# aws-neuron/neuronx-distributed

Measured on AMD Instinct MI355X. Metric: tokens/sec (whole node) Llama-2-7B training, TP=num_gpus, seq=4096, higher is better.
Workload: dtype bf16; 1 GPU; model=llama2-7b, global_batch=32, seq_len=4096, parallelism=tp1, zero1=True

## Files before the change

neuronx_distributed_amd/ops/__init__.py:

```python

import ctypes
import math
import os
from typing import Optional

import torch

_LIB = None
_LIB_ERR = None


def _load():
    global _LIB, _LIB_ERR
    if _LIB is not None or _LIB_ERR is not None:
        return _LIB
    from .build import LIB

    if not os.path.exists(LIB):
        _LIB_ERR = f"{LIB} not built — run neuronx_distributed_amd.ops.build"
        return None
    try:
        lib = ctypes.CDLL(LIB)
    except OSError as e:
        _LIB_ERR = str(e)
# ... 312 lines not shown
            dx = torch.empty_like(x)
            lib.swiglu_bwd(_ptr(x), _ptr(dy2), _ptr(dx), ctypes.c_long(N),
                           ctypes.c_int(I), _stream())
            return dx
        g, u = x[..., :I].float(), x[..., I:].float()
        dyf = dy.float()
        sig = torch.sigmoid(g)
        s = g * sig
        dg = dyf * u * (sig + s * (1 - sig))
        du = dyf * s
        return torch.cat([dg, du], dim=-1).to(x.dtype)


def swiglu(x: torch.Tensor) -> torch.Tensor:
    return _SwiGLUFn.apply(x)



def flash_attn_available() -> bool:
    lib = _load()
    return lib is not None and hasattr(lib, "flash_attn_fwd")


def _fa_ok_layout(t) -> bool:
    return t.stride(3) == 1


def _fa_strides(*tensors):
    vals = []
    for t in tensors:
        vals += [t.stride(0), t.stride(1), t.stride(2)]
    arr = (ctypes.c_long * len(vals))(*vals)
    return arr


def _fa_alloc_like(t):
    B, H, S, D = t.shape
    if t.stride(1) == D and t.stride(2) == H * D:
        return torch.empty(B, S, H, D, dtype=t.dtype,
                           device=t.device).permute(0, 2, 1, 3)
    return torch.empty_like(t, memory_format=torch.contiguous_format)


class _FlashAttnFn(torch.autograd.Function):
    @staticmethod
    def forward(ctx, q, k, v, causal, scale, window=0):
        lib = _require_lib()
        B, Hq, S, D = q.shape
        Hkv = k.shape[1]
        assert D == 128, "flash kernel supports D=128"
        assert q.dtype == torch.bfloat16
        if not _fa_ok_layout(q):
            q = q.contiguous()
        if not _fa_ok_layout(k):
            k = k.contiguous()
        if not _fa_ok_layout(v):
            v = v.contiguous()
        out = _fa_alloc_like(q)
        lse = torch.empty(B, Hq, S, dtype=torch.float32, device=q.device)
        lib.flash_attn_fwd_strided(
            _ptr(q), _ptr(k), _ptr(v), _ptr(out), _ptr(lse),
            ctypes.c_int(B), ctypes.c_int(Hq), ctypes.c_int(Hkv),
            ctypes.c_int(S), ctypes.c_float(scale),
            ctypes.c_int(1 if causal else 0), ctypes.c_int(window or 0),
            _fa_strides(q, k, v, out), _stream())
        ctx.save_for_backward(q, k, v, out, lse)
        ctx.causal = causal
        ctx.scale = scale
        ctx.window = window or 0
        return out

    @staticmethod
    def backward(ctx, dout):
        q, k, v, out, lse = ctx.saved_tensors
        lib = _require_lib()
        if not hasattr(lib, "flash_attn_bwd"):
            raise RuntimeError("flash_attn_bwd kernel not built")
        B, Hq, S, D = q.shape
        Hkv = k.shape[1]
        if not _fa_ok_layout(dout):
            dout = dout.contiguous()
        delta = torch.empty(B, Hq, S, dtype=torch.float32, device=q.device)
        dq = _fa_alloc_like(q)
        dk_pq = torch.empty(B, Hq, S, D, dtype=q.dtype, device=q.device)
        dv_pq = torch.empty(B, Hq, S, D, dtype=q.dtype, device=q.device)
        lib.flash_attn_bwd_strided(
            _ptr(q), _ptr(k), _ptr(v), _ptr(out), _ptr(dout),
            _ptr(lse), _ptr(delta), _ptr(dq), _ptr(dk_pq), _ptr(dv_pq),
            ctypes.c_int(B), ctypes.c_int(Hq), ctypes.c_int(Hkv),
            ctypes.c_int(S), ctypes.c_float(ctx.scale),
            ctypes.c_int(1 if ctx.causal else 0),
            ctypes.c_int(getattr(ctx, "window", 0)),
            _fa_strides(q, k, v, out, dout, dq, dk_pq, dv_pq), _stream())
        rep = Hq // Hkv
        if rep > 1:
            dk = dk_pq.view(B, Hkv, rep, S, D).float().sum(2).to(q.dtype)
            dv = dv_pq.view(B, Hkv, rep, S, D).float().sum(2).to(q.dtype)
        else:
            dk = dk_pq
            dv = dv_pq
        return dq, dk, dv, None, None, None


def flash_attn(q, k, v, causal=True, softmax_scale=None, window=0):
    scale = softmax_scale or 1.0 / math.sqrt(q.shape[-1])
    return _FlashAttnFn.apply(q, k, v, causal, scale, window)


def flash_attn_window_available() -> bool:
    lib = _load()
    return lib is not None and hasattr(lib, "flash_attn_fwd_window")


def flash_attn_windowed(q, k, v, window: int, softmax_scale=None):
    lib = _require_lib()
    B, Hq, S, D = q.shape
    Hkv = k.shape[1]
    assert D == 128 and q.dtype == torch.bfloat16
    scale = softmax_scale or 1.0 / math.sqrt(D)
    q, k, v = q.contiguous(), k.contiguous(), v.contiguous()
    out = torch.empty_like(q)
    lse = torch.empty(B, Hq, S, dtype=torch.float32, device=q.device)
    lib.flash_attn_fwd_window(_ptr(q), _ptr(k), _ptr(v), _ptr(out),
                              _ptr(lse), ctypes.c_int(B), ctypes.c_int(Hq),
                              ctypes.c_int(Hkv), ctypes.c_int(S),
                              ctypes.c_float(scale), ctypes.c_int(window),
                              _stream())
    return out



def adamw_step(master: torch.Tensor, m: torch.Tensor, v: torch.Tensor,
               grad_bf16: torch.Tensor, param_bf16: torch.Tensor,
               clip: Optional[torch.Tensor], lr: float, beta1: float,
               beta2: float, eps: float, weight_decay: float, step: int):
    lib = _require_lib()
    n = master.numel()
    assert m.numel() == n and v.numel() == n and grad_bf16.numel() == n
    assert grad_bf16.dtype == torch.bfloat16 and param_bf16.dtype == torch.bfloat16
    inv_bc1 = 1.0 / (1.0 - beta1 ** step)
    inv_bc2 = 1.0 / (1.0 - beta2 ** step)
    lib.adamw_step(ctypes.c_long(n), _ptr(master), _ptr(m), _ptr(v),
                   _ptr(grad_bf16), _ptr(param_bf16),
                   _ptr(clip) if clip is not None else None,
                   ctypes.c_float(lr), ctypes.c_float(beta1),
                   ctypes.c_float(beta2), ctypes.c_float(eps),
                   ctypes.c_float(weight_decay), ctypes.c_float(inv_bc1),
                   ctypes.c_float(inv_bc2), _stream())



_MOE_MB = 16


def moe_decode_available() -> bool:
    lib = _load()
    return lib is not None and hasattr(lib, "moe_decode_glu")


def moe_decode_glu(hidden: torch.Tensor, gate_up_w: torch.Tensor,
                   down_w: torch.Tensor, expert_affinities: torch.Tensor,
                   expert_index: torch.Tensor) -> torch.Tensor:
    lib = _require_lib()
    T, H = hidden.shape
    E, _, twoI = gate_up_w.shape
    I = twoI // 2
    assert H % 64 == 0 and I % 64 == 0, (H, I)
    k = expert_index.shape[1]
# ... 104 lines not shown
```

neuronx_distributed_amd/ops/csrc/flash_attn_bwd.hip:

```cpp

#include "common.h"
#include "mfma.h"

#define TR_PITCH 40

#define FA_D 128
#define LOG2E 1.4426950408889634f

extern "C" __global__ void __launch_bounds__(256)
fa_bwd_delta_kernel(const short* __restrict__ dout,
                    const short* __restrict__ out, float* __restrict__ delta,
                    long rows, int Hq, int S,
                    long do_bs, long do_hs, long do_ss,
                    long o_bs, long o_hs, long o_ss) {
  const int sub = threadIdx.x & 15;
  const long row0 = ((long)blockIdx.x * blockDim.x + threadIdx.x) >> 4;
  const long row_step = ((long)gridDim.x * blockDim.x) >> 4;
  for (long row = row0; row < rows; row += row_step) {
    const long b = row / ((long)Hq * S);
    const long h = (row / S) % Hq;
    const long sq = row % S;
    s8v dv = *(const s8v*)(dout + b * do_bs + h * do_hs + sq * do_ss
                           + sub * 8);
    s8v ov = *(const s8v*)(out + b * o_bs + h * o_hs + sq * o_ss + sub * 8);
    float s = 0.f;
#pragma unroll
    for (int j = 0; j < 8; ++j) s += bits2f(dv[j]) * bits2f(ov[j]);
#pragma unroll
    for (int off = 8; off >= 1; off >>= 1) s += __shfl_xor(s, off, 64);
    if (sub == 0) delta[row] = s;
  }
}



struct StageRegs { uint4v v0, v1; };

__device__ __forceinline__ StageRegs load_tile32(const short* __restrict__ src,
                                                 long src_row0,
                                                 long src_stride,
                                                 int rows_valid) {
  int rp = (threadIdx.x & 255) >> 4;
  int c16 = threadIdx.x & 15;
  int r0 = 2 * rp, r1 = 2 * rp + 1;
  int rr0 = r0 < rows_valid ? r0 : (rows_valid > 0 ? rows_valid - 1 : 0);
  int rr1 = r1 < rows_valid ? r1 : (rows_valid > 0 ? rows_valid - 1 : 0);
  StageRegs r;
  r.v0 = *(const uint4v*)(src + (src_row0 + rr0) * src_stride + c16 * 8);
  r.v1 = *(const uint4v*)(src + (src_row0 + rr1) * src_stride + c16 * 8);
  return r;
}

__device__ __forceinline__ void write_tile32(StageRegs r, char* lds_rm,
                                             char* lds_tr) {
  if (blockDim.x > 256 && threadIdx.x >= 256) return;
  int rp = threadIdx.x >> 4;
  int c16 = threadIdx.x & 15;
  int r0 = 2 * rp, r1 = 2 * rp + 1;
  *(uint4v*)(lds_rm + r0 * (FA_D * 2) + swz16(r0, c16 * 16)) = r.v0;
  *(uint4v*)(lds_rm + r1 * (FA_D * 2) + swz16(r1, c16 * 16)) = r.v1;
  union { uint4v u; short s[8]; } a, b;
  a.u = r.v0; b.u = r.v1;
#pragma unroll
  for (int j = 0; j < 8; ++j) {
    int d = c16 * 8 + j;
    uint pair = ((uint)(unsigned short)a.s[j]) |
                (((uint)(unsigned short)b.s[j]) << 16);
    *(uint*)(lds_tr + d * (TR_PITCH * 2) + r0 * 2) = pair;
  }
}

__device__ __forceinline__ void write_tile32_rm(StageRegs r, char* lds_rm) {
  if (blockDim.x > 256 && threadIdx.x >= 256) return;
  int rp = threadIdx.x >> 4;
  int c16 = threadIdx.x & 15;
  int r0 = 2 * rp, r1 = 2 * rp + 1;
  *(uint4v*)(lds_rm + r0 * (FA_D * 2) + swz16(r0, c16 * 16)) = r.v0;
  *(uint4v*)(lds_rm + r1 * (FA_D * 2) + swz16(r1, c16 * 16)) = r.v1;
}

__device__ __forceinline__ void stage_tile32(const short* __restrict__ src,
                                             long src_row0, long src_stride,
                                             int rows_valid, char* lds_rm,
                                             char* lds_tr) {
  if (blockDim.x > 256 && threadIdx.x >= 256) return;
  int rp = threadIdx.x >> 4;
  int c16 = threadIdx.x & 15;
  int r0 = 2 * rp, r1 = 2 * rp + 1;
  int rr0 = r0 < rows_valid ? r0 : (rows_valid > 0 ? rows_valid - 1 : 0);
  int rr1 = r1 < rows_valid ? r1 : (rows_valid > 0 ? rows_valid - 1 : 0);
  uint4v v0 = *(const uint4v*)(src + (src_row0 + rr0) * src_stride + c16 * 8);
  uint4v v1 = *(const uint4v*)(src + (src_row0 + rr1) * src_stride + c16 * 8);
  *(uint4v*)(lds_rm + r0 * (FA_D * 2) + swz16(r0, c16 * 16)) = v0;
  *(uint4v*)(lds_rm + r1 * (FA_D * 2) + swz16(r1, c16 * 16)) = v1;
  union { uint4v u; short s[8]; } a, b;
  a.u = v0; b.u = v1;
#pragma unroll
  for (int j = 0; j < 8; ++j) {
    int d = c16 * 8 + j;
    uint pair = ((uint)(unsigned short)a.s[j]) |
                (((uint)(unsigned short)b.s[j]) << 16);
    *(uint*)(lds_tr + d * (TR_PITCH * 2) + r0 * 2) = pair;
  }
}

#define TR_TILE_B (FA_D * TR_PITCH * 2)

#define TR64_PITCH 72
#define TR64_TILE_B (FA_D * TR64_PITCH * 2)
#define BW64_LDS_Q 0
#define BW64_LDS_DO (64 * FA_D * 2)
#define BW64_LDS_QT (2 * 64 * FA_D * 2)
#define BW64_LDS_DOT (2 * 64 * FA_D * 2 + TR64_TILE_B)
#define BW64_LDS_LD (2 * 64 * FA_D * 2 + 2 * TR64_TILE_B)
#define BW64_LDS_X (BW64_LDS_LD + 128 * 4)
#define BW64_X_SLOT(kvg, half, f) \
  ((((kvg) * 2 + (half)) * 4 + (f)) * 64 * 16)

struct Stage64Regs { uint4v v0, v1; };

__device__ __forceinline__ Stage64Regs load_tile64(
    const short* __restrict__ src, long src_row0, long src_stride,
    int rows_valid) {
  int rp = threadIdx.x >> 4;
  int c16 = threadIdx.x & 15;
  int r0 = 2 * rp, r1 = 2 * rp + 1;
  int rr0 = r0 < rows_valid ? r0 : (rows_valid > 0 ? rows_valid - 1 : 0);
  int rr1 = r1 < rows_valid ? r1 : (rows_valid > 0 ? rows_valid - 1 : 0);
  Stage64Regs r;
  r.v0 = *(const uint4v*)(src + (src_row0 + rr0) * src_stride + c16 * 8);
  r.v1 = *(const uint4v*)(src + (src_row0 + rr1) * src_stride + c16 * 8);
  return r;
}

__device__ __forceinline__ void write_tile64(Stage64Regs r, char* lds_rm,
                                             char* lds_tr) {
  int rp = threadIdx.x >> 4;
  int c16 = threadIdx.x & 15;
  int r0 = 2 * rp, r1 = 2 * rp + 1;
  *(uint4v*)(lds_rm + r0 * (FA_D * 2) + swz16(r0, c16 * 16)) = r.v0;
  *(uint4v*)(lds_rm + r1 * (FA_D * 2) + swz16(r1, c16 * 16)) = r.v1;
  union { uint4v u; short s[8]; } a, b;
  a.u = r.v0; b.u = r.v1;
#pragma unroll
  for (int j = 0; j < 8; ++j) {
    int d = c16 * 8 + j;
    uint pair = ((uint)(unsigned short)a.s[j]) |
                (((uint)(unsigned short)b.s[j]) << 16);
    *(uint*)(lds_tr + d * (TR64_PITCH * 2) + r0 * 2) = pair;
  }
}

__device__ __forceinline__ void stage_tile64(const short* __restrict__ src,
                                             long src_row0, long src_stride,
                                             int rows_valid, char* lds_rm,
                                             char* lds_tr) {
  write_tile64(load_tile64(src, src_row0, src_stride, rows_valid), lds_rm,
               lds_tr);
}

extern "C" __global__ void __launch_bounds__(512, 2)
fa_bwd_dkdv_kernel(const short* __restrict__ qp, const short* __restrict__ kp,
                   const short* __restrict__ vp,
                   const short* __restrict__ dop,
                   const float* __restrict__ lsep,
                   const float* __restrict__ deltap,
                   short* __restrict__ dkp, short* __restrict__ dvp,
                   int B, int Hq, int Hkv, int S, float scale, int causal,
                   int window,
                   long q_bs, long q_hs, long q_ss,
                   long k_bs, long k_hs, long k_ss,
                   long v_bs, long v_hs, long v_ss,
                   long do_bs, long do_hs, long do_ss,
                   long dk_bs, long dk_hs, long dk_ss,
                   long dv_bs, long dv_hs, long dv_ss) {
  extern __shared__ __attribute__((aligned(16))) char smem[];
  const int lane = threadIdx.x & 63;
  const int wid = __builtin_amdgcn_readfirstlane(threadIdx.x >> 6);
  const int col = lane & 31;
  const int hi = lane >> 5;
  const int kvg = wid >> 1;
  const int dhalf = wid & 1;

  const int kvblk = blockIdx.y;
  const int h = blockIdx.x;
  const int b = blockIdx.z;
  const int hkv = h / (Hq / Hkv);
  const long q_base = (long)b * q_bs + (long)h * q_hs;
  const long do_base = (long)b * do_bs + (long)h * do_hs;
  const long k_base = (long)b * k_bs + (long)hkv * k_hs;
  const long v_base = (long)b * v_bs + (long)hkv * v_hs;
  const long lse_base = (long)(b * Hq + h) * S;

  const int kv0 = kvblk * 128 + kvg * 32;
  const int my_k = kv0 + col;

  frag_u kf[8], vf[8];
  {
    int row = my_k < S ? my_k : S - 1;
#pragma unroll
    for (int c = 0; c < 8; ++c) {
      kf[c].u4 = *(const uint4v*)(kp + k_base + (long)row * k_ss + c * 16 + hi * 8);
      vf[c].u4 = *(const uint4v*)(vp + v_base + (long)row * v_ss + c * 16 + hi * 8);
    }
  }

  f32x16 dv_acc[2] = {};
  f32x16 dk_acc[2] = {};

  float* ld_sm = (float*)(smem + BW64_LDS_LD);
  auto load_ld = [&](int qt0) -> float {
    int qg = qt0 + (threadIdx.x & 63);
    int qc = qg < S ? qg : S - 1;
    if (threadIdx.x < 64) return lsep[lse_base + qc] * LOG2E;
    if (threadIdx.x < 128) return deltap[lse_base + qc];
    return 0.f;
  };
  auto write_ld = [&](float v) {
    if (threadIdx.x < 128) ld_sm[threadIdx.x] = v;
  };

  const float s2 = scale * LOG2E;
  int q_start = causal ? kvblk * 128 : 0;
  int q_end = S;
  if (window > 0) {
    int qe = kvblk * 128 + 127 + window;
    q_end = qe < S ? qe : S;
  }

  stage_tile64(qp + q_base, q_start, q_ss, S - q_start, smem + BW64_LDS_Q,
               smem + BW64_LDS_QT);
  stage_tile64(dop + do_base, q_start, do_ss, S - q_start, smem + BW64_LDS_DO,
               smem + BW64_LDS_DOT);
  write_ld(load_ld(q_start));

  Stage64Regs nq, ndo;
  float nld = 0.f;
  for (int q0 = q_start; q0 < q_end; q0 += 64) {
    __syncthreads();
    if (q0 + 64 < q_end) {
      nq = load_tile64(qp + q_base, q0 + 64, q_ss, S - q0 - 64);
      ndo = load_tile64(dop + do_base, q0 + 64, do_ss, S - q0 - 64);
      nld = load_ld(q0 + 64);
    }
    {
      const int half = dhalf;
      const int qh0 = q0 + half * 32;
      const bool produce =
          (!causal || (qh0 + 31 >= kv0)) && qh0 < S &&
          (window <= 0 || qh0 < kv0 + 31 + window);
      if (produce) {
        const int rm_row = half * 32 + col;
        const int my_kv = kv0 + col;

        f32x16 st = {};
        f32x16 dpt = {};
#pragma unroll
        for (int c = 0; c < 8; ++c) {
          frag_u qfr, dofr;
          qfr.u4 = *(const uint4v*)(smem + BW64_LDS_Q + rm_row * (FA_D * 2)
                                    + swz16(rm_row, (c * 16 + hi * 8) * 2));
          st = mfma_bf16(qfr.bf, kf[c].bf, st);
          dofr.u4 = *(const uint4v*)(smem + BW64_LDS_DO + rm_row * (FA_D * 2)
                                     + swz16(rm_row, (c * 16 + hi * 8) * 2));
          dpt = mfma_bf16(dofr.bf, vf[c].bf, dpt);
        }

        float lse_v[16], dlt_v[16];
#pragma unroll
        for (int g = 0; g < 4; ++g) {
          *(float4*)(lse_v + 4 * g) =
              *(const float4*)(ld_sm + half * 32 + 8 * g + 4 * hi);
          *(float4*)(dlt_v + 4 * g) =
              *(const float4*)(ld_sm + 64 + half * 32 + 8 * g + 4 * hi);
        }
#pragma unroll
        for (int r = 0; r < 16; ++r) {
          int ql = half * 32 + acc_row(r, hi);
          int qg = q0 + ql;
          bool masked = (causal && my_kv > qg) || my_kv >= S || qg >= S ||
              (window > 0 && qg >= my_kv + window);
          float p =
              masked ? 0.f : __builtin_amdgcn_exp2f(st[r] * s2 - lse_v[r]);
          st[r] = p;
          dpt[r] = p * (dpt[r] - dlt_v[r]);
        }

        frag_u pA[2], dA[2];
#pragma unroll
        for (int cc = 0; cc < 2; ++cc) {
          uint b0 = pack_bf16x2(st[8 * cc + 0], st[8 * cc + 1]);
          uint b1 = pack_bf16x2(st[8 * cc + 2], st[8 * cc + 3]);
          uint b2 = pack_bf16x2(st[8 * cc + 4], st[8 * cc + 5]);
          uint b3 = pack_bf16x2(st[8 * cc + 6], st[8 * cc + 7]);
          {
            auto r01 = __builtin_amdgcn_permlane32_swap(b0, b2, false, false);
            b0 = r01[0]; b2 = r01[1];
          }
          {
            auto r23 = __builtin_amdgcn_permlane32_swap(b1, b3, false, false);
            b1 = r23[0]; b3 = r23[1];
          }
          pA[cc].u[0] = b0; pA[cc].u[1] = b1;
          pA[cc].u[2] = b2; pA[cc].u[3] = b3;
          uint c0 = pack_bf16x2(dpt[8 * cc + 0], dpt[8 * cc + 1]);
          uint c1 = pack_bf16x2(dpt[8 * cc + 2], dpt[8 * cc + 3]);
          uint c2 = pack_bf16x2(dpt[8 * cc + 4], dpt[8 * cc + 5]);
          uint c3 = pack_bf16x2(dpt[8 * cc + 6], dpt[8 * cc + 7]);
          {
            auto r01 = __builtin_amdgcn_permlane32_swap(c0, c2, false, false);
            c0 = r01[0]; c2 = r01[1];
          }
          {
            auto r23 = __builtin_amdgcn_permlane32_swap(c1, c3, false, false);
            c1 = r23[0]; c3 = r23[1];
          }
          dA[cc].u[0] = c0; dA[cc].u[1] = c1;
          dA[cc].u[2] = c2; dA[cc].u[3] = c3;
        }

        char* xb = smem + BW64_LDS_X;
        *(uint4v*)(xb + BW64_X_SLOT(kvg, half, 0) + lane * 16) = pA[0].u4;
        *(uint4v*)(xb + BW64_X_SLOT(kvg, half, 1) + lane * 16) = pA[1].u4;
        *(uint4v*)(xb + BW64_X_SLOT(kvg, half, 2) + lane * 16) = dA[0].u4;
        *(uint4v*)(xb + BW64_X_SLOT(kvg, half, 3) + lane * 16) = dA[1].u4;
      }
    }
    __syncthreads();

#pragma unroll
    for (int half = 0; half < 2; ++half) {
      const int qh0 = q0 + half * 32;
      if ((causal && qh0 + 31 < kv0) || qh0 >= S ||
          (window > 0 && qh0 >= kv0 + 31 + window)) continue;

      frag_u dofr[2][2], qfr2[2][2];
#pragma unroll
      for (int cq = 0; cq < 2; ++cq)
#pragma unroll
        for (int nb = 0; nb < 2; ++nb) {
          int d = dhalf * 64 + nb * 32 + col;
          dofr[cq][nb].u4 = *(const uint4v*)(smem + BW64_LDS_DOT
                                             + d * (TR64_PITCH * 2)
                                             + (half * 32 + cq * 16 + hi * 8) * 2);
          qfr2[cq][nb].u4 = *(const uint4v*)(smem + BW64_LDS_QT
                                             + d * (TR64_PITCH * 2)
                                             + (half * 32 + cq * 16 + hi * 8) * 2);
        }
      frag_u pA[2], dA[2];
      const char* xb = smem + BW64_LDS_X;
      pA[0].u4 = *(const uint4v*)(xb + BW64_X_SLOT(kvg, half, 0) + lane * 16);
      pA[1].u4 = *(const uint4v*)(xb + BW64_X_SLOT(kvg, half, 1) + lane * 16);
      dA[0].u4 = *(const uint4v*)(xb + BW64_X_SLOT(kvg, half, 2) + lane * 16);
      dA[1].u4 = *(const uint4v*)(xb + BW64_X_SLOT(kvg, half, 3) + lane * 16);

      __builtin_amdgcn_s_setprio(1);
#pragma unroll
      for (int cq = 0; cq < 2; ++cq)
#pragma unroll
        for (int nb = 0; nb < 2; ++nb) {
          dv_acc[nb] = mfma_bf16(pA[cq].bf, dofr[cq][nb].bf, dv_acc[nb]);
          dk_acc[nb] = mfma_bf16(dA[cq].bf, qfr2[cq][nb].bf, dk_acc[nb]);
        }
      __builtin_amdgcn_s_setprio(0);
    }

    __syncthreads();
    if (q0 + 64 < q_end) {
      write_tile64(nq, smem + BW64_LDS_Q, smem + BW64_LDS_QT);
      write_tile64(ndo, smem + BW64_LDS_DO, smem + BW64_LDS_DOT);
      write_ld(nld);
    }
  }

  __syncthreads();
  char* otile = smem + wid * (32 * 64 * 2);
#pragma unroll
  for (int nb = 0; nb < 2; ++nb)
#pragma unroll
    for (int r = 0; r < 16; ++r) {
      int k = acc_row(r, hi);
      int dd = nb * 32 + col;
      *(short*)(otile + (k * 64 + dd) * 2) = f2bits(dv_acc[nb][r]);
    }
  __builtin_amdgcn_s_waitcnt(0);
#pragma unroll
  for (int i = 0; i < 4; ++i) {
    int p = lane + i * 64;
    int row = p >> 3, c16 = p & 7;
    int kg = kv0 + row;
    if (kg < S) {
      uint4v vv = *(const uint4v*)(otile + (row * 64 + c16 * 8) * 2);
      *(uint4v*)(dvp + (long)b * dv_bs + (long)h * dv_hs
                 + (long)kg * dv_ss + dhalf * 64
                 + c16 * 8) = vv;
    }
  }
  __builtin_amdgcn_s_waitcnt(0);
#pragma unroll
  for (int nb = 0; nb < 2; ++nb)
#pragma unroll
    for (int r = 0; r < 16; ++r) {
      int k = acc_row(r, hi);
      int dd = nb * 32 + col;
      *(short*)(otile + (k * 64 + dd) * 2) = f2bits(dk_acc[nb][r] * scale);
    }
  __builtin_amdgcn_s_waitcnt(0);
#pragma unroll
  for (int i = 0; i < 4; ++i) {
    int p = lane + i * 64;
    int row = p >> 3, c16 = p & 7;
    int kg = kv0 + row;
    if (kg < S) {
      uint4v vv = *(const uint4v*)(otile + (row * 64 + c16 * 8) * 2);
      *(uint4v*)(dkp + (long)b * dk_bs + (long)h * dk_hs
                 + (long)kg * dk_ss + dhalf * 64
                 + c16 * 8) = vv;
    }
  }
}

#define DQ_LDS_K 0
#define DQ_LDS_KT (32 * FA_D * 2)
#define DQ_LDS_V (32 * FA_D * 2 + TR_TILE_B)

extern "C" __global__ void __launch_bounds__(256, 2)
fa_bwd_dq_kernel(const short* __restrict__ qp, const short* __restrict__ kp,
                 const short* __restrict__ vp, const short* __restrict__ dop,
                 const float* __restrict__ lsep,
                 const float* __restrict__ deltap, short* __restrict__ dqp,
                 int B, int Hq, int Hkv, int S, float scale, int causal,
                 int window,
                 long q_bs, long q_hs, long q_ss,
                 long k_bs, long k_hs, long k_ss,
                 long v_bs, long v_hs, long v_ss,
                 long do_bs, long do_hs, long do_ss,
                 long dq_bs, long dq_hs, long dq_ss) {
  extern __shared__ __attribute__((aligned(16))) char smem[];
  const int lane = threadIdx.x & 63;
  const int wid = __builtin_amdgcn_readfirstlane(threadIdx.x >> 6);
  const int col = lane & 31;
  const int hi = lane >> 5;

  const int qblk = (int)(gridDim.y - 1 - blockIdx.y);
  const int h = blockIdx.x;
  const int b = blockIdx.z;
  const int hkv = h / (Hq / Hkv);
  const long q_base = (long)b * q_bs + (long)h * q_hs;
  const long do_base = (long)b * do_bs + (long)h * do_hs;
  const long dq_base = (long)b * dq_bs + (long)h * dq_hs;
  const long k_base = (long)b * k_bs + (long)hkv * k_hs;
  const long v_base = (long)b * v_bs + (long)hkv * v_hs;
  const long lse_base = (long)(b * Hq + h) * S;

  const int q0 = qblk * 128 + wid * 32;
  const int my_q = q0 + col;
  const int q_ld = my_q < S ? my_q : S - 1;

  frag_u qf[8], dof[8];
#pragma unroll
  for (int c = 0; c < 8; ++c) {
    qf[c].u4 = *(const uint4v*)(qp + q_base + (long)q_ld * q_ss + c * 16 + hi * 8);
    dof[c].u4 = *(const uint4v*)(dop + do_base + (long)q_ld * do_ss + c * 16 + hi * 8);
  }
  const float lse2 = lsep[lse_base + q_ld] * LOG2E;
  const float dlt = deltap[lse_base + q_ld];

  f32x16 dq_acc[4] = {};

  const int kv_end = causal ? min(S, qblk * 128 + 128) : S;
  const int kv_begin = window > 0
      ? ((qblk * 128 - window + 1 > 0 ? qblk * 128 - window + 1 : 0) & ~31)
      : 0;
  const float s2 = scale * LOG2E;

  stage_tile32(kp + k_base, kv_begin, k_ss, S - kv_begin, smem + DQ_LDS_K,
               smem + DQ_LDS_KT);
  write_tile32_rm(load_tile32(vp + v_base, kv_begin, v_ss, S - kv_begin),
                  smem + DQ_LDS_V);

  StageRegs nk, nv;
  for (int kv0 = kv_begin; kv0 < kv_end; kv0 += 32) {
    __syncthreads();
    if (kv0 + 32 < kv_end) {
      nk = load_tile32(kp + k_base, kv0 + 32, k_ss, S - kv0 - 32);
      nv = load_tile32(vp + v_base, kv0 + 32, v_ss, S - kv0 - 32);
    }
    const bool wave_active = (!causal || (kv0 <= q0 + 31)) &&
        (window <= 0 || kv0 + 31 + window > q0);

    if (wave_active) {
      f32x16 st = {};
      f32x16 dpt = {};
#pragma unroll
      for (int c = 0; c < 8; ++c) {
        frag_u kfr;
        kfr.u4 = *(const uint4v*)(smem + DQ_LDS_K + col * (FA_D * 2)
                                  + swz16(col, (c * 16 + hi * 8) * 2));
        st = mfma_bf16(kfr.bf, qf[c].bf, st);
        frag_u vfr;
        vfr.u4 = *(const uint4v*)(smem + DQ_LDS_V + col * (FA_D * 2)
                                  + swz16(col, (c * 16 + hi * 8) * 2));
        dpt = mfma_bf16(vfr.bf, dof[c].bf, dpt);
      }

      f32x16 dst;
#pragma unroll
      for (int r = 0; r < 16; ++r) {
        int kg = kv0 + acc_row(r, hi);
        bool masked = (causal && kg > my_q) || kg >= S || my_q >= S ||
            (window > 0 && kg <= my_q - window);
        float p = masked ? 0.f : __builtin_amdgcn_exp2f(st[r] * s2 - lse2);
        dst[r] = p * (dpt[r] - dlt);
      }

      frag_u kfr2[2][4];
#pragma unroll
      for (int ck = 0; ck < 2; ++ck)
#pragma unroll
        for (int nb = 0; nb < 4; ++nb) {
          int d = nb * 32 + col;
          kfr2[ck][nb].u4 = *(const uint4v*)(smem + DQ_LDS_KT
                                             + d * (TR_PITCH * 2)
                                             + (ck * 16 + hi * 8) * 2);
        }

      frag_u dA[2];
#pragma unroll
      for (int cc = 0; cc < 2; ++cc) {
        uint b0 = pack_bf16x2(dst[8 * cc + 0], dst[8 * cc + 1]);
        uint b1 = pack_bf16x2(dst[8 * cc + 2], dst[8 * cc + 3]);
        uint b2 = pack_bf16x2(dst[8 * cc + 4], dst[8 * cc + 5]);
        uint b3 = pack_bf16x2(dst[8 * cc + 6], dst[8 * cc + 7]);
        {
          auto r01 = __builtin_amdgcn_permlane32_swap(b0, b2, false, false);
          b0 = r01[0]; b2 = r01[1];
        }
        {
          auto r23 = __builtin_amdgcn_permlane32_swap(b1, b3, false, false);
          b1 = r23[0]; b3 = r23[1];
        }
        dA[cc].u[0] = b0; dA[cc].u[1] = b1;
        dA[cc].u[2] = b2; dA[cc].u[3] = b3;
      }

      __builtin_amdgcn_s_setprio(1);
#pragma unroll
      for (int ck = 0; ck < 2; ++ck) {
#pragma unroll
        for (int nb = 0; nb < 4; ++nb) {
          dq_acc[nb] = mfma_bf16(dA[ck].bf, kfr2[ck][nb].bf, dq_acc[nb]);
        }
      }
      __builtin_amdgcn_s_setprio(0);
    }

    __syncthreads();
    if (kv0 + 32 < kv_end) {
      write_tile32(nk, smem + DQ_LDS_K, smem + DQ_LDS_KT);
      write_tile32_rm(nv, smem + DQ_LDS_V);
    }
  }

  __syncthreads();
  char* otile = smem + wid * (32 * FA_D * 2);
#pragma unroll
  for (int nb = 0; nb < 4; ++nb)
#pragma unroll
    for (int r = 0; r < 16; ++r) {
      int qr = acc_row(r, hi);
      int d = nb * 32 + col;
      *(short*)(otile + (qr * FA_D + d) * 2) = f2bits(dq_acc[nb][r] * scale);
    }
  __builtin_amdgcn_s_waitcnt(0);
#pragma unroll
  for (int i = 0; i < 8; ++i) {
    int p = lane + i * 64;
    int row = p >> 4, c16 = p & 15;
    int qg = q0 + row;
    if (qg < S) {
      uint4v vv = *(const uint4v*)(otile + (row * FA_D + c16 * 8) * 2);
      *(uint4v*)(dqp + dq_base + (long)qg * dq_ss + c16 * 8) = vv;
    }
  }
}

extern "C" void flash_attn_bwd_strided(
    const void* q, const void* k, const void* v, const void* out,
    const void* dout, const void* lse, void* delta, void* dq, void* dk,
    void* dv, int B, int Hq, int Hkv, int S, float scale, int causal,
    int window, const long* st, hipStream_t stream) {
  long rows = (long)B * Hq * S;
  long blocks = (rows + 15) / 16;
  int nb = blocks < 8192 ? (int)blocks : 8192;
  fa_bwd_delta_kernel<<<nb, 256, 0, stream>>>(
      (const short*)dout, (const short*)out, (float*)delta, rows, Hq, S,
      st[12], st[13], st[14], st[9], st[10], st[11]);
  dim3 gkv(Hq, (S + 127) / 128, B);
  size_t lds1 = BW64_LDS_X + 8 * 4 * 64 * 16;
  fa_bwd_dkdv_kernel<<<gkv, 512, lds1, stream>>>(
      (const short*)q, (const short*)k, (const short*)v, (const short*)dout,
      (const float*)lse, (const float*)delta, (short*)dk, (short*)dv, B, Hq,
      Hkv, S, scale, causal, window, st[0], st[1], st[2], st[3], st[4],
      st[5], st[6], st[7], st[8], st[12], st[13], st[14], st[18], st[19],
      st[20], st[21], st[22], st[23]);
  dim3 gq(Hq, (S + 127) / 128, B);
  size_t lds2 = 4 * 32 * FA_D * 2;
  fa_bwd_dq_kernel<<<gq, 256, lds2, stream>>>(
      (const short*)q, (const short*)k, (const short*)v, (const short*)dout,
      (const float*)lse, (const float*)delta, (short*)dq, B, Hq, Hkv, S,
      scale, causal, window, st[0], st[1], st[2], st[3], st[4], st[5],
      st[6], st[7], st[8], st[12], st[13], st[14], st[15], st[16],
      st[17]);
}

extern "C" void flash_attn_bwd(const void* q, const void* k, const void* v,
                               const void* out, const void* dout,
                               const void* lse, void* delta, void* dq,
                               void* dk, void* dv, int B, int Hq, int Hkv,
                               int S, float scale, int causal,
                               hipStream_t stream) {
  const long qd[3] = {(long)Hq * S * FA_D, (long)S * FA_D, FA_D};
  const long kd[3] = {(long)Hkv * S * FA_D, (long)S * FA_D, FA_D};
  long st[24];
  for (int i = 0; i < 3; ++i) {
    st[0 + i] = qd[i];
    st[3 + i] = kd[i];
    st[6 + i] = kd[i];
    st[9 + i] = qd[i];
    st[12 + i] = qd[i];
    st[15 + i] = qd[i];
    st[18 + i] = qd[i];
    st[21 + i] = qd[i];
  }
  flash_attn_bwd_strided(q, k, v, out, dout, lse, delta, dq, dk, dv, B, Hq,
                         Hkv, S, scale, causal, 0, st, stream);
}
```

neuronx_distributed_amd/ops/csrc/mfma.h:

```cpp
#pragma once

#include "common.h"

typedef __bf16 bf16x8 __attribute__((ext_vector_type(8)));
typedef float f32x16 __attribute__((ext_vector_type(16)));
typedef unsigned int uint4v __attribute__((ext_vector_type(4)));

__device__ __forceinline__ f32x16 mfma_bf16(bf16x8 a, bf16x8 b, f32x16 c) {
  return __builtin_amdgcn_mfma_f32_32x32x16_bf16(a, b, c, 0, 0, 0);
}

union frag_u {
  bf16x8 bf;
  uint4v u4;
  uint u[4];
};

__device__ __forceinline__ int acc_row(int r, int hi) {
  return (r & 3) + 8 * (r >> 2) + 4 * hi;
}

__device__ __forceinline__ uint pack_bf16x2(float lo, float hi) {
  union { __bf16 b[2]; uint u; } r;
  r.b[0] = (__bf16)lo;
  r.b[1] = (__bf16)hi;
  return r.u;
}

__device__ __forceinline__ int swz(int row, int byte_in_row) {
  return byte_in_row ^ ((row & 7) << 4);
}

__device__ __forceinline__ int swz16(int row, int byte_in_row) {
  return byte_in_row ^ ((row & 15) << 4);
}
```

Before: 21730 tokens/s.

## Use single swizzled LDS image with transpose reads and double-buffer attention backward tiles

Replaces the separate row-major and explicitly transposed LDS copies in the flash-attention backward kernels with one swizzled tile image. Transposed operands are read with ds_read_tr16_b64, and staging buffers are double-buffered so one __syncthreads per iteration can be dropped. The dq kernel moves from 32-row to 64-row KV tiles, and masking is skipped for tiles that need no mask. It also avoids allocating per-query-head dk/dv buffers when Hq == Hkv. The aim is to cut LDS write traffic, transpose scatter stores and barriers, at the cost of more LDS per block and reliance on a new swizzle and transpose-read layout.

```diff
diff --git a/neuronx_distributed_amd/ops/__init__.py b/neuronx_distributed_amd/ops/__init__.py
--- a/neuronx_distributed_amd/ops/__init__.py
+++ b/neuronx_distributed_amd/ops/__init__.py
@@ -418,8 +418,12 @@
             dout = dout.contiguous()
         delta = torch.empty(B, Hq, S, dtype=torch.float32, device=q.device)
         dq = _fa_alloc_like(q)
-        dk_pq = torch.empty(B, Hq, S, D, dtype=q.dtype, device=q.device)
-        dv_pq = torch.empty(B, Hq, S, D, dtype=q.dtype, device=q.device)
+        if Hq == Hkv:
+            dk_pq = _fa_alloc_like(k)
+            dv_pq = _fa_alloc_like(v)
+        else:
+            dk_pq = torch.empty(B, Hq, S, D, dtype=q.dtype, device=q.device)
+            dv_pq = torch.empty(B, Hq, S, D, dtype=q.dtype, device=q.device)
         lib.flash_attn_bwd_strided(
             _ptr(q), _ptr(k), _ptr(v), _ptr(out), _ptr(dout),
             _ptr(lse), _ptr(delta), _ptr(dq), _ptr(dk_pq), _ptr(dv_pq),
diff --git a/neuronx_distributed_amd/ops/csrc/flash_attn_bwd.hip b/neuronx_distributed_amd/ops/csrc/flash_attn_bwd.hip
--- a/neuronx_distributed_amd/ops/csrc/flash_attn_bwd.hip
+++ b/neuronx_distributed_amd/ops/csrc/flash_attn_bwd.hip
@@ -1,8 +1,6 @@
 
 #include "common.h"
 #include "mfma.h"
-
-#define TR_PITCH 40
 
 #define FA_D 128
 #define LOG2E 1.4426950408889634f
@@ -33,131 +31,45 @@
 }
 
 
-
-struct StageRegs { uint4v v0, v1; };
-
-__device__ __forceinline__ StageRegs load_tile32(const short* __restrict__ src,
-                                                 long src_row0,
-                                                 long src_stride,
-                                                 int rows_valid) {
-  int rp = (threadIdx.x & 255) >> 4;
-  int c16 = threadIdx.x & 15;
-  int r0 = 2 * rp, r1 = 2 * rp + 1;
-  int rr0 = r0 < rows_valid ? r0 : (rows_valid > 0 ? rows_valid - 1 : 0);
-  int rr1 = r1 < rows_valid ? r1 : (rows_valid > 0 ? rows_valid - 1 : 0);
-  StageRegs r;
-  r.v0 = *(const uint4v*)(src + (src_row0 + rr0) * src_stride + c16 * 8);
-  r.v1 = *(const uint4v*)(src + (src_row0 + rr1) * src_stride + c16 * 8);
+#define TILE64_B (64 * IMG_ROW_B)
+
+template <int NR>
+struct StageRegs { uint4v v[NR]; };
+
+template <int NR>
+__device__ __forceinline__ StageRegs<NR> load_tile64(
+    const short* __restrict__ src, long src_row0, long src_stride,
+    int rows_valid) {
+  const int rp = threadIdx.x >> 4;
+  const int c16 = threadIdx.x & 15;
+  const int last = rows_valid > 0 ? rows_valid - 1 : 0;
+  StageRegs<NR> r;
+#pragma unroll
+  for (int i = 0; i < NR; ++i) {
+    int row = NR * rp + i;
+    int rr = row < rows_valid ? row : last;
+    r.v[i] = *(const uint4v*)(src + (src_row0 + rr) * src_stride + c16 * 8);
+  }
   return r;
 }
 
-__device__ __forceinline__ void write_tile32(StageRegs r, char* lds_rm,
-                                             char* lds_tr) {
-  if (blockDim.x > 256 && threadIdx.x >= 256) return;
-  int rp = threadIdx.x >> 4;
-  int c16 = threadIdx.x & 15;
-  int r0 = 2 * rp, r1 = 2 * rp + 1;
-  *(uint4v*)(lds_rm + r0 * (FA_D * 2) + swz16(r0, c16 * 16)) = r.v0;
-  *(uint4v*)(lds_rm + r1 * (FA_D * 2) + swz16(r1, c16 * 16)) = r.v1;
-  union { uint4v u; short s[8]; } a, b;
-  a.u = r.v0; b.u = r.v1;
-#pragma unroll
-  for (int j = 0; j < 8; ++j) {
-    int d = c16 * 8 + j;
-    uint pair = ((uint)(unsigned short)a.s[j]) |
-                (((uint)(unsigned short)b.s[j]) << 16);
-    *(uint*)(lds_tr + d * (TR_PITCH * 2) + r0 * 2) = pair;
-  }
-}
-
-__device__ __forceinline__ void write_tile32_rm(StageRegs r, char* lds_rm) {
-  if (blockDim.x > 256 && threadIdx.x >= 256) return;
-  int rp = threadIdx.x >> 4;
-  int c16 = threadIdx.x & 15;
-  int r0 = 2 * rp, r1 = 2 * rp + 1;
-  *(uint4v*)(lds_rm + r0 * (FA_D * 2) + swz16(r0, c16 * 16)) = r.v0;
-  *(uint4v*)(lds_rm + r1 * (FA_D * 2) + swz16(r1, c16 * 16)) = r.v1;
-}
-
-__device__ __forceinline__ void stage_tile32(const short* __restrict__ src,
-                                             long src_row0, long src_stride,
-                                             int rows_valid, char* lds_rm,
-                                             char* lds_tr) {
-  if (blockDim.x > 256 && threadIdx.x >= 256) return;
-  int rp = threadIdx.x >> 4;
-  int c16 = threadIdx.x & 15;
-  int r0 = 2 * rp, r1 = 2 * rp + 1;
-  int rr0 = r0 < rows_valid ? r0 : (rows_valid > 0 ? rows_valid - 1 : 0);
-  int rr1 = r1 < rows_valid ? r1 : (rows_valid > 0 ? rows_valid - 1 : 0);
-  uint4v v0 = *(const uint4v*)(src + (src_row0 + rr0) * src_stride + c16 * 8);
-  uint4v v1 = *(const uint4v*)(src + (src_row0 + rr1) * src_stride + c16 * 8);
-  *(uint4v*)(lds_rm + r0 * (FA_D * 2) + swz16(r0, c16 * 16)) = v0;
-  *(uint4v*)(lds_rm + r1 * (FA_D * 2) + swz16(r1, c16 * 16)) = v1;
-  union { uint4v u; short s[8]; } a, b;
-  a.u = v0; b.u = v1;
-#pragma unroll
-  for (int j = 0; j < 8; ++j) {
-    int d = c16 * 8 + j;
-    uint pair = ((uint)(unsigned short)a.s[j]) |
-                (((uint)(unsigned short)b.s[j]) << 16);
-    *(uint*)(lds_tr + d * (TR_PITCH * 2) + r0 * 2) = pair;
-  }
-}
-
-#define TR_TILE_B (FA_D * TR_PITCH * 2)
-
-#define TR64_PITCH 72
-#define TR64_TILE_B (FA_D * TR64_PITCH * 2)
+template <int NR>
+__device__ __forceinline__ void write_tile64(StageRegs<NR> r, char* img) {
+  const int rp = threadIdx.x >> 4;
+  const int c16 = threadIdx.x & 15;
+#pragma unroll
+  for (int i = 0; i < NR; ++i)
+    *(uint4v*)(img + img_off(NR * rp + i, c16)) = r.v[i];
+}
+
+#define BW64_BUF_B (2 * TILE64_B + 128 * 4)
 #define BW64_LDS_Q 0
-#define BW64_LDS_DO (64 * FA_D * 2)
-#define BW64_LDS_QT (2 * 64 * FA_D * 2)
-#define BW64_LDS_DOT (2 * 64 * FA_D * 2 + TR64_TILE_B)
-#define BW64_LDS_LD (2 * 64 * FA_D * 2 + 2 * TR64_TILE_B)
-#define BW64_LDS_X (BW64_LDS_LD + 128 * 4)
+#define BW64_LDS_DO TILE64_B
+#define BW64_LDS_LD (2 * TILE64_B)
+#define BW64_LDS_X (2 * BW64_BUF_B)
 #define BW64_X_SLOT(kvg, half, f) \
   ((((kvg) * 2 + (half)) * 4 + (f)) * 64 * 16)
-
-struct Stage64Regs { uint4v v0, v1; };
-
-__device__ __forceinline__ Stage64Regs load_tile64(
-    const short* __restrict__ src, long src_row0, long src_stride,
-    int rows_valid) {
-  int rp = threadIdx.x >> 4;
-  int c16 = threadIdx.x & 15;
-  int r0 = 2 * rp, r1 = 2 * rp + 1;
-  int rr0 = r0 < rows_valid ? r0 : (rows_valid > 0 ? rows_valid - 1 : 0);
-  int rr1 = r1 < rows_valid ? r1 : (rows_valid > 0 ? rows_valid - 1 : 0);
-  Stage64Regs r;
-  r.v0 = *(const uint4v*)(src + (src_row0 + rr0) * src_stride + c16 * 8);
-  r.v1 = *(const uint4v*)(src + (src_row0 + rr1) * src_stride + c16 * 8);
-  return r;
-}
-
-__device__ __forceinline__ void write_tile64(Stage64Regs r, char* lds_rm,
-                                             char* lds_tr) {
-  int rp = threadIdx.x >> 4;
-  int c16 = threadIdx.x & 15;
-  int r0 = 2 * rp, r1 = 2 * rp + 1;
-  *(uint4v*)(lds_rm + r0 * (FA_D * 2) + swz16(r0, c16 * 16)) = r.v0;
-  *(uint4v*)(lds_rm + r1 * (FA_D * 2) + swz16(r1, c16 * 16)) = r.v1;
-  union { uint4v u; short s[8]; } a, b;
-  a.u = r.v0; b.u = r.v1;
-#pragma unroll
-  for (int j = 0; j < 8; ++j) {
-    int d = c16 * 8 + j;
-    uint pair = ((uint)(unsigned short)a.s[j]) |
-                (((uint)(unsigned short)b.s[j]) << 16);
-    *(uint*)(lds_tr + d * (TR64_PITCH * 2) + r0 * 2) = pair;
-  }
-}
-
-__device__ __forceinline__ void stage_tile64(const short* __restrict__ src,
-                                             long src_row0, long src_stride,
-                                             int rows_valid, char* lds_rm,
-                                             char* lds_tr) {
-  write_tile64(load_tile64(src, src_row0, src_stride, rows_valid), lds_rm,
-               lds_tr);
-}
+#define BW64_LDS_TOTAL (BW64_LDS_X + 8 * 4 * 64 * 16)
 
 extern "C" __global__ void __launch_bounds__(512, 2)
 fa_bwd_dkdv_kernel(const short* __restrict__ qp, const short* __restrict__ kp,
@@ -208,7 +120,6 @@
   f32x16 dv_acc[2] = {};
   f32x16 dk_acc[2] = {};
 
-  float* ld_sm = (float*)(smem + BW64_LDS_LD);
   auto load_ld = [&](int qt0) -> float {
     int qg = qt0 + (threadIdx.x & 63);
     int qc = qg < S ? qg : S - 1;
@@ -216,8 +127,8 @@
     if (threadIdx.x < 128) return deltap[lse_base + qc];
     return 0.f;
   };
-  auto write_ld = [&](float v) {
-    if (threadIdx.x < 128) ld_sm[threadIdx.x] = v;
+  auto write_ld = [&](float v, char* buf) {
+    if (threadIdx.x < 128) ((float*)(buf + BW64_LDS_LD))[threadIdx.x] = v;
   };
 
   const float s2 = scale * LOG2E;
@@ -228,19 +139,26 @@
     q_end = qe < S ? qe : S;
   }
 
-  stage_tile64(qp + q_base, q_start, q_ss, S - q_start, smem + BW64_LDS_Q,
-               smem + BW64_LDS_QT);
-  stage_tile64(dop + do_base, q_start, do_ss, S - q_start, smem + BW64_LDS_DO,
-               smem + BW64_LDS_DOT);
-  write_ld(load_ld(q_start));
-
-  Stage64Regs nq, ndo;
+  write_tile64(load_tile64<2>(qp + q_base, q_start, q_ss, S - q_start),
+               smem + BW64_LDS_Q);
+  write_tile64(load_tile64<2>(dop + do_base, q_start, do_ss, S - q_start),
+               smem + BW64_LDS_DO);
+  write_ld(load_ld(q_start), smem);
+
+  const int row_base = img_row_base(col, hi);
+  const int tr_base = img_tr_base(lane) ^ (dhalf * 128);
+  StageRegs<2> nq, ndo;
   float nld = 0.f;
-  for (int q0 = q_start; q0 < q_end; q0 += 64) {
+  int cur = 0;
+  for (int q0 = q_start; q0 < q_end; q0 += 64, cur ^= 1) {
+    const int sb_off = cur * BW64_BUF_B;
+    const float* ld_sm = (const float*)(smem + sb_off + BW64_LDS_LD);
+    const int rowb = row_base + sb_off;
+    const int trb = tr_base + sb_off;
     __syncthreads();
     if (q0 + 64 < q_end) {
-      nq = load_tile64(qp + q_base, q0 + 64, q_ss, S - q0 - 64);
-      ndo = load_tile64(dop + do_base, q0 + 64, do_ss, S - q0 - 64);
+      nq = load_tile64<2>(qp + q_base, q0 + 64, q_ss, S - q0 - 64);
+      ndo = load_tile64<2>(dop + do_base, q0 + 64, do_ss, S - q0 - 64);
       nld = load_ld(q0 + 64);
     }
     {
@@ -250,7 +168,6 @@
           (!causal || (qh0 + 31 >= kv0)) && qh0 < S &&
           (window <= 0 || qh0 < kv0 + 31 + window);
       if (produce) {
-        const int rm_row = half * 32 + col;
         const int my_kv = kv0 + col;
 
         f32x16 st = {};
@@ -258,11 +175,9 @@
 #pragma unroll
         for (int c = 0; c < 8; ++c) {
           frag_u qfr, dofr;
-          qfr.u4 = *(const uint4v*)(smem + BW64_LDS_Q + rm_row * (FA_D * 2)
-                                    + swz16(rm_row, (c * 16 + hi * 8) * 2));
+          qfr.u4 = img_row_read(smem + BW64_LDS_Q, rowb + half * (32 * IMG_ROW_B), c);
           st = mfma_bf16(qfr.bf, kf[c].bf, st);
-          dofr.u4 = *(const uint4v*)(smem + BW64_LDS_DO + rm_row * (FA_D * 2)
-                                     + swz16(rm_row, (c * 16 + hi * 8) * 2));
+          dofr.u4 = img_row_read(smem + BW64_LDS_DO, rowb + half * (32 * IMG_ROW_B), c);
           dpt = mfma_bf16(dofr.bf, vf[c].bf, dpt);
         }
 
@@ -274,17 +189,24 @@
           *(float4*)(dlt_v + 4 * g) =
               *(const float4*)(ld_sm + 64 + half * 32 + 8 * g + 4 * hi);
         }
-#pragma unroll
-        for (int r = 0; r < 16; ++r) {
-          int ql = half * 32 + acc_row(r, hi);
-          int qg = q0 + ql;
-          bool masked = (causal && my_kv > qg) || my_kv >= S || qg >= S ||
-              (window > 0 && qg >= my_kv + window);
-          float p =
-              masked ? 0.f : __builtin_amdgcn_exp2f(st[r] * s2 - lse_v[r]);
-          st[r] = p;
-          dpt[r] = p * (dpt[r] - dlt_v[r]);
-        }
+        const bool need_mask =
+            (causal && kv0 + 31 > qh0) || kv0 + 31 >= S || qh0 + 31 >= S ||
+            (window > 0 && qh0 + 31 >= kv0 + window);
+#pragma unroll
+        for (int r = 0; r < 16; ++r)
+          st[r] = __builtin_amdgcn_exp2f(st[r] * s2 - lse_v[r]);
+        if (need_mask) {
+#pragma unroll
+          for (int r = 0; r < 16; ++r) {
+            int ql = half * 32 + acc_row(r, hi);
+            int qg = q0 + ql;
+            bool masked = ((causal != 0) & (my_kv > qg)) | (my_kv >= S) |
+                (qg >= S) | ((window > 0) & (qg >= my_kv + window));
+            st[r] = masked ? 0.f : st[r];
+          }
+        }
+#pragma unroll
+        for (int r = 0; r < 16; ++r) dpt[r] = st[r] * (dpt[r] - dlt_v[r]);
 
         frag_u pA[2], dA[2];
 #pragma unroll
@@ -339,13 +261,10 @@
       for (int cq = 0; cq < 2; ++cq)
 #pragma unroll
         for (int nb = 0; nb < 2; ++nb) {
-          int d = dhalf * 64 + nb * 32 + col;
-          dofr[cq][nb].u4 = *(const uint4v*)(smem + BW64_LDS_DOT
-                                             + d * (TR64_PITCH * 2)
-                                             + (half * 32 + cq * 16 + hi * 8) * 2);
-          qfr2[cq][nb].u4 = *(const uint4v*)(smem + BW64_LDS_QT
-                                             + d * (TR64_PITCH * 2)
-                                             + (half * 32 + cq * 16 + hi * 8) * 2);
+          dofr[cq][nb].u4 = img_tr_read(smem + BW64_LDS_DO, trb,
+                                        half * 32 + cq * 16, nb * 32);
+          qfr2[cq][nb].u4 = img_tr_read(smem + BW64_LDS_Q, trb,
+                                        half * 32 + cq * 16, nb * 32);
         }
       frag_u pA[2], dA[2];
       const char* xb = smem + BW64_LDS_X;
@@ -365,11 +284,11 @@
       __builtin_amdgcn_s_setprio(0);
     }
 
-    __syncthreads();
     if (q0 + 64 < q_end) {
-      write_tile64(nq, smem + BW64_LDS_Q, smem + BW64_LDS_QT);
-      write_tile64(ndo, smem + BW64_LDS_DO, smem + BW64_LDS_DOT);
-      write_ld(nld);
+      char* nxt = smem + (cur ^ 1) * BW64_BUF_B;
+      write_tile64(nq, nxt + BW64_LDS_Q);
+      write_tile64(ndo, nxt + BW64_LDS_DO);
+      write_ld(nld, nxt);
     }
   }
 
@@ -420,9 +339,10 @@
   }
 }
 
+#define DQ_BUF_B (2 * TILE64_B)
 #define DQ_LDS_K 0
-#define DQ_LDS_KT (32 * FA_D * 2)
-#define DQ_LDS_V (32 * FA_D * 2 + TR_TILE_B)
+#define DQ_LDS_V TILE64_B
+#define DQ_LDS_TOTAL (2 * DQ_BUF_B)
 
 extern "C" __global__ void __launch_bounds__(256, 2)
 fa_bwd_dq_kernel(const short* __restrict__ qp, const short* __restrict__ kp,
@@ -474,56 +394,69 @@
       : 0;
   const float s2 = scale * LOG2E;
 
-  stage_tile32(kp + k_base, kv_begin, k_ss, S - kv_begin, smem + DQ_LDS_K,
-               smem + DQ_LDS_KT);
-  write_tile32_rm(load_tile32(vp + v_base, kv_begin, v_ss, S - kv_begin),
-                  smem + DQ_LDS_V);
-
-  StageRegs nk, nv;
-  for (int kv0 = kv_begin; kv0 < kv_end; kv0 += 32) {
+  write_tile64(load_tile64<4>(kp + k_base, kv_begin, k_ss, S - kv_begin),
+               smem + DQ_LDS_K);
+  write_tile64(load_tile64<4>(vp + v_base, kv_begin, v_ss, S - kv_begin),
+               smem + DQ_LDS_V);
+
+  const int row_base = img_row_base(col, hi);
+  const int tr_base = img_tr_base(lane);
+  StageRegs<4> nk, nv;
+  int cur = 0;
+  for (int kv0 = kv_begin; kv0 < kv_end; kv0 += 64, cur ^= 1) {
+    const int rowb = row_base + cur * DQ_BUF_B;
+    const int trb = tr_base + cur * DQ_BUF_B;
     __syncthreads();
-    if (kv0 + 32 < kv_end) {
-      nk = load_tile32(kp + k_base, kv0 + 32, k_ss, S - kv0 - 32);
-      nv = load_tile32(vp + v_base, kv0 + 32, v_ss, S - kv0 - 32);
-    }
-    const bool wave_active = (!causal || (kv0 <= q0 + 31)) &&
-        (window <= 0 || kv0 + 31 + window > q0);
-
-    if (wave_active) {
+    if (kv0 + 64 < kv_end) {
+      nk = load_tile64<4>(kp + k_base, kv0 + 64, k_ss, S - kv0 - 64);
+      nv = load_tile64<4>(vp + v_base, kv0 + 64, v_ss, S - kv0 - 64);
+    }
+#pragma unroll
+    for (int half = 0; half < 2; ++half) {
+      const int kvh0 = kv0 + half * 32;
+      const bool wave_active = kvh0 < kv_end &&
+          (!causal || (kvh0 <= q0 + 31)) &&
+          (window <= 0 || kvh0 + 31 + window > q0);
+      if (!wave_active) continue;
+
       f32x16 st = {};
       f32x16 dpt = {};
 #pragma unroll
       for (int c = 0; c < 8; ++c) {
         frag_u kfr;
-        kfr.u4 = *(const uint4v*)(smem + DQ_LDS_K + col * (FA_D * 2)
-                                  + swz16(col, (c * 16 + hi * 8) * 2));
+        kfr.u4 = img_row_read(smem + DQ_LDS_K, rowb + half * (32 * IMG_ROW_B), c);
         st = mfma_bf16(kfr.bf, qf[c].bf, st);
         frag_u vfr;
-        vfr.u4 = *(const uint4v*)(smem + DQ_LDS_V + col * (FA_D * 2)
-                                  + swz16(col, (c * 16 + hi * 8) * 2));
+        vfr.u4 = img_row_read(smem + DQ_LDS_V, rowb + half * (32 * IMG_ROW_B), c);
         dpt = mfma_bf16(vfr.bf, dof[c].bf, dpt);
       }
 
+      const bool need_mask =
+          (causal && kvh0 + 31 > q0) || kvh0 + 31 >= S || q0 + 31 >= S ||
+          (window > 0 && kvh0 <= q0 + 31 - window);
+#pragma unroll
+      for (int r = 0; r < 16; ++r)
+        st[r] = __builtin_amdgcn_exp2f(st[r] * s2 - lse2);
+      if (need_mask) {
+#pragma unroll
+        for (int r = 0; r < 16; ++r) {
+          int kg = kvh0 + acc_row(r, hi);
+          bool masked = ((causal != 0) & (kg > my_q)) | (kg >= S) |
+              (my_q >= S) | ((window > 0) & (kg <= my_q - window));
+          st[r] = masked ? 0.f : st[r];
+        }
+      }
       f32x16 dst;
 #pragma unroll
-      for (int r = 0; r < 16; ++r) {
-        int kg = kv0 + acc_row(r, hi);
-        bool masked = (causal && kg > my_q) || kg >= S || my_q >= S ||
-            (window > 0 && kg <= my_q - window);
-        float p = masked ? 0.f : __builtin_amdgcn_exp2f(st[r] * s2 - lse2);
-        dst[r] = p * (dpt[r] - dlt);
-      }
+      for (int r = 0; r < 16; ++r) dst[r] = st[r] * (dpt[r] - dlt);
 
       frag_u kfr2[2][4];
 #pragma unroll
       for (int ck = 0; ck < 2; ++ck)
 #pragma unroll
-        for (int nb = 0; nb < 4; ++nb) {
-          int d = nb * 32 + col;
-          kfr2[ck][nb].u4 = *(const uint4v*)(smem + DQ_LDS_KT
-                                             + d * (TR_PITCH * 2)
-                                             + (ck * 16 + hi * 8) * 2);
-        }
+        for (int nb = 0; nb < 4; ++nb)
+          kfr2[ck][nb].u4 = img_tr_read(smem + DQ_LDS_K, trb,
+                                        half * 32 + ck * 16, nb * 32);
 
       frag_u dA[2];
 #pragma unroll
@@ -555,10 +488,10 @@
       __builtin_amdgcn_s_setprio(0);
     }
 
-    __syncthreads();
-    if (kv0 + 32 < kv_end) {
-      write_tile32(nk, smem + DQ_LDS_K, smem + DQ_LDS_KT);
-      write_tile32_rm(nv, smem + DQ_LDS_V);
+    if (kv0 + 64 < kv_end) {
+      char* nxt = smem + (cur ^ 1) * DQ_BUF_B;
+      write_tile64(nk, nxt + DQ_LDS_K);
+      write_tile64(nv, nxt + DQ_LDS_V);
     }
   }
 
@@ -597,7 +530,7 @@
       (const short*)dout, (const short*)out, (float*)delta, rows, Hq, S,
       st[12], st[13], st[14], st[9], st[10], st[11]);
   dim3 gkv(Hq, (S + 127) / 128, B);
-  size_t lds1 = BW64_LDS_X + 8 * 4 * 64 * 16;
+  size_t lds1 = BW64_LDS_TOTAL;
   fa_bwd_dkdv_kernel<<<gkv, 512, lds1, stream>>>(
       (const short*)q, (const short*)k, (const short*)v, (const short*)dout,
       (const float*)lse, (const float*)delta, (short*)dk, (short*)dv, B, Hq,
@@ -605,7 +538,7 @@
       st[5], st[6], st[7], st[8], st[12], st[13], st[14], st[18], st[19],
       st[20], st[21], st[22], st[23]);
   dim3 gq(Hq, (S + 127) / 128, B);
-  size_t lds2 = 4 * 32 * FA_D * 2;
+  size_t lds2 = DQ_LDS_TOTAL;
   fa_bwd_dq_kernel<<<gq, 256, lds2, stream>>>(
       (const short*)q, (const short*)k, (const short*)v, (const short*)dout,
       (const float*)lse, (const float*)delta, (short*)dq, B, Hq, Hkv, S,
diff --git a/neuronx_distributed_amd/ops/csrc/mfma.h b/neuronx_distributed_amd/ops/csrc/mfma.h
--- a/neuronx_distributed_amd/ops/csrc/mfma.h
+++ b/neuronx_distributed_amd/ops/csrc/mfma.h
@@ -34,3 +34,36 @@
 __device__ __forceinline__ int swz16(int row, int byte_in_row) {
   return byte_in_row ^ ((row & 15) << 4);
 }
+
+#define IMG_ROW_B 256
+
+__device__ __forceinline__ int img_off(int row, int ch) {
+  return IMG_ROW_B * row + 16 * (ch ^ (((row & 3) << 2) | ((row >> 2) & 3)));
+}
+
+
+__device__ __forceinline__ int img_row_base(int row, int hi) {
+  return img_off(row, hi);
+}
+__device__ __forceinline__ uint4v img_row_read(const char* img, int base,
+                                               int c) {
+  return *(const uint4v*)(img + (base ^ (32 * c)));
+}
+
+typedef short s4v_t __attribute__((ext_vector_type(4)));
+__device__ __forceinline__ int img_tr_base(int lane) {
+  const int i = lane & 15;
+  const int q = i >> 2, p = i & 3;
+  return img_off(8 * (lane >> 5) + q, 2 * ((lane >> 4) & 1) + (p >> 1)) +
+         8 * (p & 1);
+}
+__device__ __forceinline__ uint4v img_tr_read(const char* img, int base,
+                                              int k0, int n0) {
+  typedef __attribute__((address_space(3))) s4v_t lds_s4v;
+  union { s4v_t s[2]; uint4v u4; } r;
+  r.s[0] = __builtin_amdgcn_ds_read_tr16_b64_v4i16(
+      (lds_s4v*)(img + (base ^ (2 * n0)) + IMG_ROW_B * k0));
+  r.s[1] = __builtin_amdgcn_ds_read_tr16_b64_v4i16(
+      (lds_s4v*)(img + (base ^ (2 * n0) ^ 16) + IMG_ROW_B * (k0 + 4)));
+  return r.u4;
+}
diff --git a/neuronx_distributed_amd/ops/csrc/probe_lds_image.hip b/neuronx_distributed_amd/ops/csrc/probe_lds_image.hip
--- /dev/null
+++ b/neuronx_distributed_amd/ops/csrc/probe_lds_image.hip
@@ -0,0 +1,37 @@
+
+#include "common.h"
+#include "mfma.h"
+
+extern "C" __global__ void __launch_bounds__(64)
+probe_lds_image_kernel(const short* __restrict__ tile,
+                       short* __restrict__ row_out,
+                       short* __restrict__ tr_out) {
+  extern __shared__ __attribute__((aligned(16))) char smem[];
+  const int lane = threadIdx.x & 63;
+  const int col = lane & 31;
+  const int hi = lane >> 5;
+#pragma unroll
+  for (int i = 0; i < 8; ++i) {
+    int p = lane + i * 64;
+    int row = p >> 4, ch = p & 15;
+    *(uint4v*)(smem + img_off(row, ch)) =
+        *(const uint4v*)(tile + row * 128 + ch * 8);
+  }
+  __syncthreads();
+#pragma unroll
+  for (int c = 0; c < 8; ++c)
+    *(uint4v*)(row_out + (c * 64 + lane) * 8) =
+        img_row_read(smem, img_row_base(col, hi), c);
+#pragma unroll
+  for (int ck = 0; ck < 2; ++ck)
+#pragma unroll
+    for (int nb = 0; nb < 4; ++nb)
+      *(uint4v*)(tr_out + ((ck * 4 + nb) * 64 + lane) * 8) =
+          img_tr_read(smem, img_tr_base(lane), ck * 16, nb * 32);
+}
+
+extern "C" void run_probe_lds_image(const void* tile, void* row_out,
+                                    void* tr_out, hipStream_t s) {
+  probe_lds_image_kernel<<<1, 64, 32 * IMG_ROW_B, s>>>(
+      (const short*)tile, (short*)row_out, (short*)tr_out);
+}
```

Result: faster. 23950 tokens/s, median of 6 (+10.2%).
